# REXJJ/depth-map-fusion-utils

Measured on AMD Instinct MI355X. Metric: ray-voxel updates/sec (3D-DDA log-odds fusion, 512^3 grid, 640x480 depth), higher is better.
Workload: dtype int32

## Files before the change

### depth-map-fusion-utils_amd/csrc/dmf_brick.hpp

```cpp
#pragma once
#include <cmath>
#include <cstdint>

#ifndef __HIPCC__
#define __host__
#define __device__
#endif

namespace dmf {
namespace brick {

constexpr int kLog = 5;
constexpr int kB = 1 << kLog;
constexpr int kCells = kB * kB * kB;
constexpr int kMaxBricks = 32768;
constexpr int64_t kQ = 256;
constexpr int32_t kNever = 1 << 30;
constexpr int64_t kNever64 = (int64_t)1 << 62;

struct QRay {
  int32_t cs[3], ce[3];
  int32_t st[3];
  int32_t n[3];
  int32_t adq[3];
  int32_t h0[3];
  int32_t nsteps;
  bool end_inside;
};

__host__ __device__ inline void pack_ray(const int64_t qs[3], const int64_t qe[3], bool end_inside, uint64_t& A,
                                         uint64_t& B) {
  A = (uint64_t)qs[0] | ((uint64_t)qs[1] << 19) | ((uint64_t)qs[2] << 38) | ((uint64_t)(end_inside ? 1 : 0) << 63);
  B = (uint64_t)qe[0] | ((uint64_t)qe[1] << 19) | ((uint64_t)qe[2] << 38) | ((uint64_t)1 << 63);
}

__host__ __device__ inline void qray_from(const int32_t qs[3], const int32_t qe[3], bool end_inside, QRay& r) {
  r.end_inside = end_inside;
  r.nsteps = 0;
#pragma unroll
  for (int a = 0; a < 3; ++a) {
    r.cs[a] = qs[a] >> 8;
    r.ce[a] = qe[a] >> 8;
    const int32_t dq = qe[a] - qs[a];
    r.adq[a] = dq < 0 ? -dq : dq;
    r.st[a] = r.ce[a] > r.cs[a] ? 1 : (r.ce[a] < r.cs[a] ? -1 : 0);
    r.n[a] = r.ce[a] > r.cs[a] ? r.ce[a] - r.cs[a] : r.cs[a] - r.ce[a];
    r.h0[a] = r.st[a] > 0 ? 2 * ((r.cs[a] + 1) * (int32_t)kQ - qs[a]) : 2 * (qs[a] - r.cs[a] * (int32_t)kQ) + 1;
    r.nsteps += r.n[a];
  }
}

__host__ __device__ inline void decode_ray(uint64_t A, uint64_t B, QRay& r) {
  constexpr uint64_t m = (1u << 19) - 1;
  const int32_t qs[3] = {(int32_t)(A & m), (int32_t)((A >> 19) & m), (int32_t)((A >> 38) & m)};
  const int32_t qe[3] = {(int32_t)(B & m), (int32_t)((B >> 19) & m), (int32_t)((B >> 38) & m)};
  qray_from(qs, qe, (A >> 63) != 0, r);
}

__host__ __device__ inline int32_t e0_pair(const QRay& r, int a, int b) {
  if (r.st[a] && r.st[b]) return (int32_t)((int64_t)r.h0[a] * r.adq[b] - (int64_t)r.h0[b] * r.adq[a]);
  return r.st[a] ? -kNever : (r.st[b] ? kNever : 0);
}

__host__ __device__ inline bool ev_before(const QRay& r, int a, int64_t Ha, int b, int64_t Hb) {
  const int64_t L = Ha * (int64_t)r.adq[b], R = Hb * (int64_t)r.adq[a];
  return L < R || (L == R && a < b);
}

__host__ __device__ inline int32_t quot_small32(int64_t X, int32_t Y) {
  const float xf = (float)(int32_t)(X >> 20) * 1048576.0f + (float)(int32_t)(X & 0xfffff);
  const float yf = (float)Y;
#if defined(__HIP_DEVICE_COMPILE__)
  int32_t q = (int32_t)(xf * __builtin_amdgcn_rcpf(yf));
#else
  int32_t q = (int32_t)(xf / yf);
#endif
  const int32_t rm = (int32_t)((uint32_t)X - (uint32_t)q * (uint32_t)Y);
  q += rm < 0 ? -1 : (rm >= Y ? 1 : 0);
  return q;
}

__host__ __device__ inline int32_t count_at(const QRay& r, int b, int a, int32_t Ha) {
  if (r.st[b] == 0) return 0;
  const int64_t X = (int64_t)Ha * (int64_t)r.adq[b] - (int64_t)r.h0[b] * (int64_t)r.adq[a];
  const int32_t Y = (int32_t)(2 * kQ) * r.adq[a];
  int32_t c;
  if (b < a) c = X < 0 ? 0 : quot_small32(X, Y) + 1;
  else c = X <= 0 ? 0 : quot_small32(X - 1, Y) + 1;
  return c < r.n[b] ? c : r.n[b];
}

__host__ __device__ inline void counts_at(const QRay& r, int a, int32_t k, int32_t c[3]) {
  if (a < 0) { c[0] = c[1] = c[2] = 0; return; }
  const int32_t Ha = r.h0[a] + (int32_t)(2 * kQ) * k;
#pragma unroll
  for (int b = 0; b < 3; ++b) c[b] = (b == a) ? k + 1 : count_at(r, b, a, Ha);
}

__host__ __device__ inline int32_t opaque(int32_t x) {
#if defined(__HIP_DEVICE_COMPILE__)
  asm("" : "+v"(x));
#endif
  return x;
}

#if defined(__HIP_DEVICE_COMPILE__)
extern "C" __device__ int32_t dmf_llvm_mul_i24(int32_t, int32_t) __asm("llvm.amdgcn.mul.i24");
#endif
__host__ __device__ inline int32_t mul24(int32_t a, int32_t b) {
#if defined(__HIP_DEVICE_COMPILE__)
  return dmf_llvm_mul_i24(a, b);
#else
  return (int32_t)((uint32_t)a * (uint32_t)b);
#endif
}

__host__ __device__ inline int32_t sel3(bool a0, bool a1, int32_t v0, int32_t v1, int32_t v2) {
  return a0 ? opaque(v0) : (a1 ? opaque(v1) : opaque(v2));
}

__host__ __device__ inline void counts_at_sel(const QRay& r, int a, int32_t k, int32_t c[3]) {
  const bool a0 = a == 0, a1 = a == 1, a2 = a == 2;
  const int32_t ha = sel3(a0, a1, r.h0[0], r.h0[1], r.h0[2]);
  const int32_t da = sel3(a0, a1, r.adq[0], r.adq[1], r.adq[2]);
  const int64_t Ha = (int64_t)ha + 2 * kQ * (int64_t)k;
  const int32_t Y = (int32_t)(2 * kQ) * da;
  auto cnt = [&](int32_t adb, int32_t hb, int32_t nb, bool after) -> int32_t {
    const int64_t X = Ha * (int64_t)adb - (int64_t)hb * (int64_t)da - (after ? 1 : 0);
    const int32_t q = quot_small32(X < 0 ? 0 : X, Y) + 1;
    return X < 0 ? 0 : (q < 0 ? 0 : (q > nb ? nb : q));
  };
  const int32_t c1 = cnt(a0 ? opaque(r.adq[1]) : opaque(r.adq[0]), a0 ? opaque(r.h0[1]) : opaque(r.h0[0]),
// ... 10 lines not shown
  double hx[3][3];
};
__host__ __device__ inline void qray_f64(const QRay& r, QRayF64& f) {
#pragma unroll
  for (int a = 0; a < 3; ++a) {
    f.adq[a] = (double)r.adq[a];
    f.h[a] = (double)r.h0[a];
#if defined(__HIP_DEVICE_COMPILE__)
    f.inv[a] = r.adq[a] ? __builtin_amdgcn_rcp(2.0 * (double)kQ * (double)r.adq[a]) : 0.0;
#else
    f.inv[a] = r.adq[a] ? 1.0 / (2.0 * (double)kQ * (double)r.adq[a]) : 0.0;
#endif
  }
#pragma unroll
  for (int a = 0; a < 3; ++a)
#pragma unroll
    for (int b = 0; b < 3; ++b) f.hx[a][b] = -(f.h[b] * f.adq[a]) - (b > a ? 1.0 : 0.0);
}
template <int A>
__host__ __device__ inline void counts_at_f64(const QRay& r, const QRayF64& f, int32_t k, int32_t c[3]) {
  const double Ha = fma(2.0 * (double)kQ, (double)k, f.h[A]);
  const double Y = 2.0 * (double)kQ * f.adq[A];
#pragma unroll
  for (int b = 0; b < 3; ++b) {
    if (b == A) {
      c[b] = k + 1;
      continue;
    }
    const double X = fma(Ha, f.adq[b], f.hx[A][b]);
    const double q = floor(X * f.inv[A]);
    const double rm = fma(-q, Y, X);
    const int32_t cq = (int32_t)q + (rm < 0.0 ? 0 : 1) + (rm >= Y ? 1 : 0);
    c[b] = (r.st[b] == 0 || X < 0.0) ? 0 : (cq < r.n[b] ? cq : r.n[b]);
  }
}

struct Pair {
  int32_t cin[3];
  int32_t cells;
  bool ends;
};

__host__ __device__ inline void pair_in_brick(const QRay& r, const int32_t bb[3], const int32_t ng[3], Pair& p) {
  int ai = -1, ao = -1;
  int32_t ki = 0, ko = 0;
  int64_t Hi = 0, Ho = 0;
#pragma unroll
  for (int a = 0; a < 3; ++a) {
    const int32_t lo = bb[a] << kLog;
    const int32_t hi = (lo + kB - 1 < ng[a] - 1) ? lo + kB - 1 : ng[a] - 1;
    int32_t k = -1;
    if (r.st[a] > 0 && r.cs[a] < lo) k = lo - r.cs[a] - 1;
    if (r.st[a] < 0 && r.cs[a] > hi) k = r.cs[a] - hi - 1;
    if (k >= 0) {
      const int64_t H = (int64_t)r.h0[a] + 2 * kQ * (int64_t)k;
      if (ai < 0 || ev_before(r, ai, Hi, a, H)) { ai = a; ki = k; Hi = H; }
    }
    k = -1;
    if (r.st[a] > 0 && r.ce[a] > hi) k = hi - r.cs[a];
    if (r.st[a] < 0 && r.ce[a] < lo) k = r.cs[a] - lo;
    if (k >= 0) {
      const int64_t H = (int64_t)r.h0[a] + 2 * kQ * (int64_t)k;
      if (ao < 0 || ev_before(r, a, H, ao, Ho)) { ao = a; ko = k; Ho = H; }
    }
  }
  counts_at(r, ai, ki, p.cin);
  const int32_t idx_in = p.cin[0] + p.cin[1] + p.cin[2];
  if (ao >= 0) {
    int32_t co[3];
    counts_at(r, ao, ko, co);
    p.cells = co[0] + co[1] + co[2] - idx_in;
    p.ends = false;
  } else {
    p.cells = r.nsteps - idx_in + 1;
    p.ends = true;
  }
}

struct Coarse {
  int64_t E01, E02, E12, K0, K1, K2;
  int32_t total;
};

__host__ __device__ inline int32_t coarse_total(const QRay& r) {
  int32_t total = 0;
#pragma unroll
  for (int a = 0; a < 3; ++a) {
    const int32_t off = r.cs[a] & (kB - 1);
    const int32_t k0 = r.st[a] > 0 ? kB - 1 - off : off;
    if (r.st[a] != 0 && r.n[a] > k0) total += (r.n[a] - 1 - k0) / kB + 1;
  }
  return total;
}

__host__ __device__ inline void coarse_init(const QRay& r, Coarse& w) {
  int32_t H[3];
  w.total = coarse_total(r);
#pragma unroll
  for (int a = 0; a < 3; ++a) {
    const int32_t off = r.cs[a] & (kB - 1);
    const int32_t k0 = r.st[a] > 0 ? kB - 1 - off : off;
    H[a] = r.h0[a] + (int32_t)(2 * kQ) * k0;
  }
  auto pr = [&](int a, int b) -> int64_t {
    if (r.st[a] && r.st[b]) return (int64_t)H[a] * (int64_t)r.adq[b] - (int64_t)H[b] * (int64_t)r.adq[a];
    return r.st[a] ? -kNever64 : (r.st[b] ? kNever64 : 0);
  };
  w.E01 = pr(0, 1);
  w.E02 = pr(0, 2);
  w.E12 = pr(1, 2);
  w.K0 = (int64_t)kB * 2 * kQ * r.adq[0];
  w.K1 = (int64_t)kB * 2 * kQ * r.adq[1];
  w.K2 = (int64_t)kB * 2 * kQ * r.adq[2];
}

__host__ __device__ inline int coarse_next(Coarse& w) {
  const bool b10 = w.E01 > 0;
  const bool s2 = (b10 ? w.E12 : w.E02) > 0;
  const bool s1 = !s2 && b10, s0 = !s2 && !b10;
  w.E01 += s0 ? w.K1 : (s1 ? -w.K0 : 0);
  w.E02 += s0 ? w.K2 : (s2 ? -w.K0 : 0);
  w.E12 += s1 ? w.K2 : (s2 ? -w.K1 : 0);
  return s2 ? 2 : (s1 ? 1 : 0);
}

static_assert(kB * 2 * kQ == (1 << (kLog + 9)), "coarse K = 2^(kLog + 9) |dq|");
constexpr int kCoarseShift = kLog + 9;
constexpr int32_t kNever32 = 1 << 30;
struct Coarse32 {
  int32_t g01, g02, g12;
  int32_t d0, d1, d2;
  int32_t total;
};

__host__ __device__ inline void coarse_init32(const QRay& r, Coarse32& w) {
  int32_t H[3];
  w.total = coarse_total(r);
#pragma unroll
  for (int a = 0; a < 3; ++a) {
    const int32_t off = r.cs[a] & (kB - 1);
    const int32_t k0 = r.st[a] > 0 ? kB - 1 - off : off;
    H[a] = r.h0[a] + (int32_t)(2 * kQ) * k0;
  }
  auto pr = [&](int a, int b) -> int32_t {
    if (r.st[a] && r.st[b]) {
      auto mul = [](int32_t x, int32_t y) {
        return (int64_t)((uint64_t)((uint32_t)x & 0xffffffu) * ((uint32_t)y & 0xffffffu));
      };
      const int64_t E = mul(H[a], r.adq[b]) - mul(H[b], r.adq[a]);
      return (int32_t)((E - 1) >> kCoarseShift);
    }
    return r.st[a] ? -kNever32 : (r.st[b] ? kNever32 : -1);
  };
  w.g01 = pr(0, 1);
  w.g02 = pr(0, 2);
  w.g12 = pr(1, 2);
  w.d0 = r.adq[0];
  w.d1 = r.adq[1];
  w.d2 = r.adq[2];
}

__host__ __device__ inline int coarse_next32(Coarse32& w) {
  const bool b10 = w.g01 >= 0;
  const bool s2 = (b10 ? w.g12 : w.g02) >= 0;
  const bool s1 = !s2 && b10, s0 = !s2 && !b10;
  w.g01 += s0 ? w.d1 : (s1 ? -w.d0 : 0);
  w.g02 += s0 ? w.d2 : (s2 ? -w.d0 : 0);
  w.g12 += s1 ? w.d2 : (s2 ? -w.d1 : 0);
  return s2 ? 2 : (s1 ? 1 : 0);
}

__host__ __device__ inline bool coarse_gamma_ok(const QRay& r, const Coarse32& w) {
  auto ok = [&](int a, int b, int32_t g) {
    if (!r.st[a] || !r.st[b]) return true;
    const int32_t m = (r.adq[a] > r.adq[b] ? r.adq[a] : r.adq[b]) + 1;
    return g <= m && g >= -m;
  };
  return ok(0, 1, w.g01) && ok(0, 2, w.g02) && ok(1, 2, w.g12);
}

__host__ __device__ inline int32_t pinned(int32_t x) {
#if defined(__HIP_DEVICE_COMPILE__)
  asm volatile("" : "+v"(x));
#endif
  return x;
}
__host__ __device__ inline int coarse_next_k(const QRay& r, int32_t k0, int32_t k1, int32_t k2) {
  int best = -1;
  int64_t Hb = 0;
  int32_t db = 0;
  const int32_t ks[3] = {k0, k1, k2};
#pragma unroll
  for (int a = 0; a < 3; ++a) {
    const int32_t st = pinned(r.st[a]);
    if (st == 0) continue;
    const int32_t da = pinned(r.adq[a]);
    const int64_t H = (int64_t)pinned(r.h0[a]) + 2 * kQ * (int64_t)ks[a];
    if (best < 0 || H * (int64_t)db < Hb * (int64_t)da) {
      best = a;
      Hb = H;
      db = da;
    }
  }
  return best;
}
__host__ __device__ inline int32_t next_boundary_k(const QRay& r, int a, int b) {
  const int32_t st = r.st[a], nb = b + st;
  return st > 0 ? nb * kB - r.cs[a] - 1 : r.cs[a] - nb * kB - kB;
}
__host__ __device__ inline int coarse_next_at(const QRay& r, int b0, int b1, int b2) {
  return coarse_next_k(r, next_boundary_k(r, 0, b0), next_boundary_k(r, 1, b1), next_boundary_k(r, 2, b2));
}

constexpr int kPathSteps = 32;
__host__ __device__ inline uint64_t path_put(uint64_t path, int t, int a) {
  return t < kPathSteps ? path | (uint64_t)a << (2 * t) : path;
}
__host__ __device__ inline int path_axis(uint64_t path, int t) { return (int)(path >> (2 * t)) & 3; }
__host__ __device__ inline uint32_t path_word_put(uint32_t word, int t, int a) {
  return word | (uint32_t)a << ((2 * t) & 31);
}
__host__ __device__ inline int wave_uniform(int x) {
#if defined(__HIP_DEVICE_COMPILE__)
  return __builtin_amdgcn_readfirstlane(x);
// ... 231 lines not shown
```

### depth-map-fusion-utils_amd/csrc/dmf_dda.hpp

```cpp
#pragma once
#include "dmf_internal.hpp"

namespace dmf {

constexpr int64_t kQ = 256;

__device__ inline int64_t clampi(int64_t v, int64_t lo, int64_t hi) { return v < lo ? lo : (v > hi ? hi : v); }
__device__ inline int32_t clamp32(int32_t v, int32_t lo, int32_t hi) { return v < lo ? lo : (v > hi ? hi : v); }

__device__ inline int32_t floor_sat32(double x) {
  const double f = floor(x);
  return fabs(f) < 9223372036854775808.0 ? (int32_t)fmin(fmax(f, -1073741824.0), 1073741824.0) : -(1 << 30);
}

__device__ inline void atomic_add_dev(int32_t* p, int32_t v) {
  __hip_atomic_fetch_add(p, v, __ATOMIC_RELAXED, __HIP_MEMORY_SCOPE_AGENT);
}

struct Tiles {
  uint32_t ny, nz;
};
__host__ __device__ inline Tiles tiles_of(const int n[3]) {
  return Tiles{(uint32_t)(n[1] + 1) >> 1, (uint32_t)(n[2] + 3) >> 2};
}
__host__ __device__ inline uint32_t tile_base(const Tiles& t, int tx, int ty, int tz) {
  return (((uint32_t)tx * t.ny + (uint32_t)ty) * t.nz + (uint32_t)tz) << 4;
}
__host__ __device__ inline uint32_t tiled_index(const Tiles& t, int x, int y, int z) {
  return tile_base(t, x >> 1, y >> 1, z >> 2) | (uint32_t)(((x & 1) << 3) | ((y & 1) << 2) | (z & 3));
}
inline size_t tiled_cells(const int n[3]) {
  return (size_t)((n[0] + 1) >> 1) * (size_t)((n[1] + 1) >> 1) * (size_t)((n[2] + 3) >> 2) * 16;
}

struct Ray {
  int c[3];
  int st[3];
  int32_t E01, E02, E12;
  int32_t K[3];
  int left;
  bool end_inside;
};
constexpr int32_t kNever = 1 << 30;

__device__ inline void dda_select(int32_t& E01, int32_t& E02, int32_t& E12, int32_t K0, int32_t K1, int32_t K2,
                                  bool& s0, bool& s1, bool& s2) {
  const bool b10 = E01 > 0;
  s2 = (b10 ? E12 : E02) > 0;
  s1 = !s2 && b10;
  s0 = !s2 && !b10;
  E01 += s0 ? K1 : (s1 ? -K0 : 0);
  E02 += s0 ? K2 : (s2 ? -K0 : 0);
  E12 += s1 ? K2 : (s2 ? -K1 : 0);
}

struct Walk {
  int c0, c1, c2, st0, st1, st2;
  int32_t E01, E02, E12, K0, K1, K2;
  int left;
  __device__ explicit Walk(const Ray& R)
      : c0(R.c[0]), c1(R.c[1]), c2(R.c[2]), st0(R.st[0]), st1(R.st[1]), st2(R.st[2]), E01(R.E01), E02(R.E02),
        E12(R.E12), K0(R.K[0]), K1(R.K[1]), K2(R.K[2]), left(R.left) {}
  __device__ void step() {
    bool s0, s1, s2;
    dda_select(E01, E02, E12, K0, K1, K2, s0, s1, s2);
    c0 += s0 ? st0 : 0;
    c1 += s1 ? st1 : 0;
    c2 += s2 ? st2 : 0;
  }
};

__device__ inline double grid_coord(const Geom& g, int a, float x) {
  const double t = (double)x - g.mn[a];
  return g.pow2 ? t * g.inv[a] : t / g.dl[a];
}

__device__ inline void grid_origin(const Geom& g, const float O[3], double go[3]) {
#pragma unroll
  for (int a = 0; a < 3; ++a) go[a] = grid_coord(g, a, O[a]);
}

__device__ inline bool dda_quantize_go(const Geom& g, const double go[3], const float E[3], bool end_inside,
                                       int64_t qs[3], int64_t qe[3]) {
  double ge[3], D[3];
#pragma unroll
  for (int a = 0; a < 3; ++a) {
    ge[a] = grid_coord(g, a, E[a]);
    D[a] = ge[a] - go[a];
  }
  double t0 = 0.0, t1 = 1.0;
#pragma unroll
  for (int a = 0; a < 3; ++a) {
    if (D[a] == 0.0) {
      if (go[a] < 0.0 || go[a] >= (double)g.n[a]) return false;
    } else if (end_inside) {
      if (D[a] > 0.0 ? go[a] < 0.0 : go[a] > (double)g.n[a]) {
        const double lo = (D[a] > 0.0 ? 0.0 - go[a] : (double)g.n[a] - go[a]) / D[a];
        if (lo > t0) t0 = lo;
      }
    } else {
      double ta = (0.0 - go[a]) / D[a];
      double tb = ((double)g.n[a] - go[a]) / D[a];
      if (ta > tb) { const double tt = ta; ta = tb; tb = tt; }
      if (ta > t0) t0 = ta;
      if (tb < t1) t1 = tb;
    }
  }
  if (end_inside) { t1 = 1.0; if (t0 > 1.0) t0 = 1.0; }
  if (t0 > t1) return false;
#pragma unroll
  for (int a = 0; a < 3; ++a) {
    const double gs = go[a] + t0 * D[a];
    const double gx = end_inside ? ge[a] : go[a] + t1 * D[a];
    const int32_t n = (int32_t)g.n[a], Q = (int32_t)kQ;
    const int32_t cs = clamp32(floor_sat32(gs), 0, n - 1);
    const int32_t ce = end_inside ? floor_sat32(ge[a]) : clamp32(floor_sat32(gx), 0, n - 1);
    qs[a] = clamp32(floor_sat32(gs * (double)kQ), cs * Q, cs * Q + Q - 1);
    qe[a] = clamp32(floor_sat32(gx * (double)kQ), ce * Q, ce * Q + Q - 1);
  }
  return true;
}

__device__ inline bool dda_quantize(const Geom& g, const float O[3], const float E[3], bool end_inside, int64_t qs[3],
                                    int64_t qe[3]) {
  double go[3];
  grid_origin(g, O, go);
  return dda_quantize_go(g, go, E, end_inside, qs, qe);
}

__device__ inline bool dda_setup(const Geom& g, const float O[3], const float E[3], bool end_inside, Ray& R) {
  int64_t qs[3], qe[3];
  if (!dda_quantize(g, O, E, end_inside, qs, qe)) return false;
  int64_t cs[3], ce[3];
#pragma unroll
  for (int a = 0; a < 3; ++a) {
    cs[a] = qs[a] / kQ;
    ce[a] = qe[a] / kQ;
  }
  int64_t adq[3], h[3];
#pragma unroll
  for (int a = 0; a < 3; ++a) {
    const int64_t dq = qe[a] - qs[a];
    adq[a] = dq < 0 ? -dq : dq;
    R.st[a] = ce[a] > cs[a] ? 1 : (ce[a] < cs[a] ? -1 : 0);
    h[a] = R.st[a] > 0 ? 2 * ((cs[a] + 1) * kQ - qs[a]) : 2 * (qs[a] - cs[a] * kQ) + 1;
    R.K[a] = (int32_t)(2 * kQ * adq[a]);
  }
  auto pair = [&](int a, int b) -> int32_t {
    if (R.st[a] && R.st[b]) return (int32_t)(h[a] * adq[b] - h[b] * adq[a]);
    return R.st[a] ? -kNever : (R.st[b] ? kNever : 0);
  };
  R.E01 = pair(0, 1);
  R.E02 = pair(0, 2);
  R.E12 = pair(1, 2);
  const int nsteps = (int)((ce[0] > cs[0] ? ce[0] - cs[0] : cs[0] - ce[0]) + (ce[1] > cs[1] ? ce[1] - cs[1] : cs[1] - ce[1]) +
                           (ce[2] > cs[2] ? ce[2] - cs[2] : cs[2] - ce[2]));
  R.c[0] = (int)cs[0];
  R.c[1] = (int)cs[1];
  R.c[2] = (int)cs[2];
  R.left = nsteps + 1;
  R.end_inside = end_inside;
  return true;
}

__device__ inline bool endpoint_inside(const Geom& g, const float E[3]) {
  const bool in = (E[0] >= g.vlo[0]) & (E[0] <= g.vhi[0]) & (E[1] >= g.vlo[1]) & (E[1] <= g.vhi[1]) &
                  (E[2] >= g.vlo[2]) & (E[2] <= g.vhi[2]);
  if (!in) return false;
  return valid_coords(g, bin_axis(g, 0, E[0]), bin_axis(g, 1, E[1]), bin_axis(g, 2, E[2]));
}

__device__ inline int pixel_ray(const Geom& g, const CamP& cam, const uint16_t* __restrict__ depth,
                                const PoseX* __restrict__ poses, int p, int r, int c, int dmin, int dmax, Ray& R,
                                bool& valid) {
  R.left = 0;
  valid = false;
  if (r >= cam.H || c >= cam.W) return 0;
  const int d = depth[((int64_t)p * cam.H + r) * cam.W + c];
  if (!(d >= dmin && d < dmax)) return 0;
  valid = true;
  const PoseX& T = poses[p];
  float pc[3], E[3];
  project(cam, r, c, d, pc);
  xform(T.f, pc[0], pc[1], pc[2], E);
  const bool inside = endpoint_inside(g, E);
  const float O[3] = {T.f[3], T.f[7], T.f[11]};
  if (!dda_setup(g, O, E, inside, R)) { R.left = 0; return 0; }
  return R.left;
}

__device__ inline bool pixel_quant_go(const Geom& g, const CamP& cam, int d, const float Tf[12], const double go[3],
                                      int r, int c, int dmin, int dmax, int64_t qs[3], int64_t qe[3], bool& inside,
                                      bool& valid) {
  valid = false;
  inside = false;
  if (d < 0 || !(d >= dmin && d < dmax)) return false;
  valid = true;
  float pc[3], E[3];
  project(cam, r, c, d, pc);
  xform(Tf, pc[0], pc[1], pc[2], E);
  inside = endpoint_inside(g, E);
  return dda_quantize_go(g, go, E, inside, qs, qe);
}

__device__ inline int pixel_depth(const CamP& cam, const uint16_t* __restrict__ depth, int p, int r, int c) {
  return (r >= cam.H || c >= cam.W) ? -1 : (int)depth[((int64_t)p * cam.H + r) * cam.W + c];
}

__device__ inline int32_t rc_div(int64_t x, int32_t k) {
  int32_t q = (int32_t)((float)x * __builtin_amdgcn_rcpf((float)k));
  int64_t r = x - (int64_t)q * k;
  if (r < 0) { --q; r += k; }
  if (r < 0) { --q; r += k; }
  if (r >= k) { ++q; r -= k; }
  if (r >= k) { ++q; }
  return q;
}

__device__ inline int rc_jump(int m, Walk& W) {
  const int r0 = W.st0 > 0 ? m - (W.c0 & m) : (W.st0 < 0 ? (W.c0 & m) : 0);
  const int r1 = W.st1 > 0 ? m - (W.c1 & m) : (W.st1 < 0 ? (W.c1 & m) : 0);
  const int r2 = W.st2 > 0 ? m - (W.c2 & m) : (W.st2 < 0 ? (W.c2 & m) : 0);
  const int64_t F01 = (int64_t)W.E01 + (int64_t)r0 * W.K1 - (int64_t)r1 * W.K0;
  const int64_t F02 = (int64_t)W.E02 + (int64_t)r0 * W.K2 - (int64_t)r2 * W.K0;
  const int64_t F12 = (int64_t)W.E12 + (int64_t)r1 * W.K2 - (int64_t)r2 * W.K1;
  const bool b10 = F01 > 0;
  const bool s2 = (b10 ? F12 : F02) > 0, s1 = !s2 && b10;
  auto before = [](int64_t d, int rs, int32_t kb, int32_t ka, bool b_after) -> int {
    const int64_t x = d + (int64_t)rs * kb;
    if (x < 0 || ka == 0) return 0;
    const int32_t q = rc_div(x, ka);
    return b_after ? (int)(q + ((int64_t)q * ka < x ? 1 : 0)) : (int)q + 1;
  };
  int n0, n1, n2;
  if (s2) {
    n2 = r2 + 1;
    n0 = before(-(int64_t)W.E02, r2, W.K0, W.K2, false);
    n1 = before(-(int64_t)W.E12, r2, W.K1, W.K2, false);
  } else if (s1) {
    n1 = r1 + 1;
    n0 = before(-(int64_t)W.E01, r1, W.K0, W.K1, false);
    n2 = before((int64_t)W.E12, r1, W.K2, W.K1, true);
  } else {
    n0 = r0 + 1;
    n1 = before((int64_t)W.E01, r0, W.K1, W.K0, true);
    n2 = before((int64_t)W.E02, r0, W.K2, W.K0, true);
  }
  W.c0 += W.st0 * n0;
  W.c1 += W.st1 * n1;
  W.c2 += W.st2 * n2;
  W.E01 = (int32_t)((uint32_t)W.E01 + (uint32_t)n0 * (uint32_t)W.K1 - (uint32_t)n1 * (uint32_t)W.K0);
  W.E02 = (int32_t)((uint32_t)W.E02 + (uint32_t)n0 * (uint32_t)W.K2 - (uint32_t)n2 * (uint32_t)W.K0);
  W.E12 = (int32_t)((uint32_t)W.E12 + (uint32_t)n1 * (uint32_t)W.K2 - (uint32_t)n2 * (uint32_t)W.K1);
  return n0 + n1 + n2;
}

}
```

### depth-map-fusion-utils_amd/csrc/dmf_fuse.hip

```cpp
#include <algorithm>
#include <atomic>
#include <cmath>
#include <cstdlib>
#include <string>
#include <type_traits>

#include "dmf_brick.hpp"
#include "dmf_dda.hpp"
#include "dmf_host.hpp"

namespace dmf {

struct DepthSrc {
  CamP cam;
  const uint16_t* depth;
  const PoseX* poses;
  int dmin, dmax, packets_x;
  struct Frame { float Tf[12]; };
  struct Sample { int d, r, c; };
  __device__ void begin(const Geom& g, int p, Frame& f, double go[3]) const {
#pragma unroll
    for (int i = 0; i < 12; ++i) f.Tf[i] = poses[p].f[i];
    const float O[3] = {f.Tf[3], f.Tf[7], f.Tf[11]};
    grid_origin(g, O, go);
  }
  __device__ Sample load(int p, int q, int l) const {
    Sample s;
    s.r = (q / packets_x) * 8 + (l >> 3);
    s.c = (q % packets_x) * 8 + (l & 7);
    s.d = pixel_depth(cam, depth, p, s.r, s.c);
    return s;
  }
  __device__ bool quant(const Geom& g, const Frame& f, const double go[3], const Sample& s, int64_t qs[3],
                        int64_t qe[3], bool& inside, bool& valid) const {
    return pixel_quant_go(g, cam, s.d, f.Tf, go, s.r, s.c, dmin, dmax, qs, qe, inside, valid);
  }
  __device__ int ray(const Geom& g, int p, int q, int l, Ray& R, bool& valid) const {
    return pixel_ray(g, cam, depth, poses, p, (q / packets_x) * 8 + (l >> 3), (q % packets_x) * 8 + (l & 7), dmin,
                     dmax, R, valid);
  }
};

struct PointSrc {
  const float* xyz;
  const float* origins;
  int64_t N;
  struct Frame { bool live; };
  struct Sample { float E[3]; bool ok; };
  __device__ static bool finite3(const float v[3]) {
    return __builtin_isfinite(v[0]) & __builtin_isfinite(v[1]) & __builtin_isfinite(v[2]);
  }
  __device__ void origin(int p, float O[3]) const {
    const float* const o = origins + 3 * (int64_t)p;
    O[0] = o[0];
    O[1] = o[1];
    O[2] = o[2];
  }
  __device__ void begin(const Geom& g, int p, Frame& f, double go[3]) const {
    float O[3];
    origin(p, O);
    f.live = finite3(O);
    grid_origin(g, O, go);
  }
  __device__ Sample load(int p, int q, int l) const {
    Sample s;
    const int64_t i = (int64_t)q * 64 + l;
    s.ok = i < N;
    const float* const e = xyz + ((int64_t)p * N + (s.ok ? i : 0)) * 3;
    s.E[0] = e[0];
    s.E[1] = e[1];
    s.E[2] = e[2];
    return s;
  }
  __device__ bool quant(const Geom& g, const Frame& f, const double go[3], const Sample& s, int64_t qs[3],
                        int64_t qe[3], bool& inside, bool& valid) const {
    inside = false;
    valid = f.live & s.ok & finite3(s.E);
    if (!valid) return false;
    inside = endpoint_inside(g, s.E);
    return dda_quantize_go(g, go, s.E, inside, qs, qe);
  }
  __device__ int ray(const Geom& g, int p, int q, int l, Ray& R, bool& valid) const {
    float O[3];
    origin(p, O);
    const Sample s = load(p, q, l);
    R.left = 0;
    valid = finite3(O) && s.ok && finite3(s.E);
    if (!valid) return 0;
    if (!dda_setup(g, O, s.E, endpoint_inside(g, s.E), R)) { R.left = 0; return 0; }
    return R.left;
  }
};

__device__ inline void wave_stats(unsigned long long* stats, unsigned long long upd, unsigned long long ray,
                                  unsigned long long hit) {
  for (int o = 32; o > 0; o >>= 1) {
    upd += __shfl_down(upd, o, 64);
    ray += __shfl_down(ray, o, 64);
    hit += __shfl_down(hit, o, 64);
  }
  if ((threadIdx.x & 63) == 0) {
    if (upd) atomicAdd(&stats[0], upd);
    if (ray) atomicAdd(&stats[1], ray);
    if (hit) atomicAdd(&stats[2], hit);
  }
}


typedef unsigned short us2 __attribute__((ext_vector_type(2)));
__device__ inline uint32_t pkmax(uint32_t a, uint32_t b) {
  us2 x = __builtin_bit_cast(us2, a), y = __builtin_bit_cast(us2, b);
  return __builtin_bit_cast(uint32_t, __builtin_elementwise_max(x, y));
}
__device__ inline uint32_t wave_pkmax(uint32_t v) {
  v = pkmax(v, (uint32_t)__builtin_amdgcn_update_dpp(0, (int)v, 0x111, 0xf, 0xf, false));
  v = pkmax(v, (uint32_t)__builtin_amdgcn_update_dpp(0, (int)v, 0x112, 0xf, 0xf, false));
  v = pkmax(v, (uint32_t)__builtin_amdgcn_update_dpp(0, (int)v, 0x114, 0xf, 0xf, false));
  v = pkmax(v, (uint32_t)__builtin_amdgcn_update_dpp(0, (int)v, 0x118, 0xf, 0xf, false));
  v = pkmax(v, (uint32_t)__builtin_amdgcn_update_dpp(0, (int)v, 0x142, 0xa, 0xf, false));
  v = pkmax(v, (uint32_t)__builtin_amdgcn_update_dpp(0, (int)v, 0x143, 0xc, 0xf, false));
  return (uint32_t)__builtin_amdgcn_readlane((int)v, 63);
}

__device__ inline int lane_prefix(uint64_t mask) {
  return (int)__builtin_amdgcn_mbcnt_hi((uint32_t)(mask >> 32), __builtin_amdgcn_mbcnt_lo((uint32_t)mask, 0u));
}

__device__ inline int small_div(int i, int b, float rb, int& rem) {
  int q = (int)((float)i * rb);
  int r = i - q * b;
  if (r < 0) { --q; r += b; }
  if (r >= b) { ++q; r -= b; }
  rem = r;
  return q;
}

__device__ inline int popc(uint32_t v) { return __builtin_popcount(v); }
__device__ inline int popc(uint64_t v) { return __builtin_popcountll(v); }

template <int kS, int kBox, class Src>
__global__ __launch_bounds__(64) void k_fuse_l(Geom g, Src src, int32_t* __restrict__ hits,
                                               int32_t* __restrict__ misses,
                                               unsigned long long* __restrict__ stats) {
  static_assert(kS <= 31, "2-bit codes of up to 31 advances with a 64-bit field mask");
  using CodeT = typename std::conditional<(kS <= 15), uint32_t, uint64_t>::type;
  constexpr CodeT kOne = 1, kOdd = (CodeT)0x5555555555555555ull, kEven = (CodeT)0xAAAAAAAAAAAAAAAAull;
  static_assert(kBox % 256 == 0 && kBox <= 65536, "box scanned 256 cells per iteration, 16-bit indices");
  static_assert(kBox >= 64 * kS, "the non-zero list lives in the box");
  stats = stat_slot(stats);
  __shared__ __attribute__((aligned(16))) int box[kBox];
  uint32_t* nzl = (uint32_t*)box;
  const int l = threadIdx.x;
  for (int i = l; i < kBox; i += 64) box[i] = 0;
  const Tiles tl = tiles_of(g.n);
  Ray R;
  bool valid;
  const unsigned long long upd = (unsigned long long)src.ray(g, (int)blockIdx.y, (int)blockIdx.x, l, R, valid);
  const unsigned long long nvalid = valid ? 1 : 0, nhit = (R.left > 0 && R.end_inside) ? 1 : 0;
  int32_t E01 = R.E01, E02 = R.E02, E12 = R.E12;
  const int32_t K0 = R.K[0], K1 = R.K[1], K2 = R.K[2];
  const int st0 = R.st[0], st1 = R.st[1], st2 = R.st[2];
  int c0 = R.c[0], c1 = R.c[1], c2 = R.c[2], left = R.left;
  const bool end_inside = R.end_inside;
// ... 149 lines not shown

template <class F>
__device__ inline uint64_t bk_coarse(const BkGeom& bg, const bk::QRay& R, F&& f) {
  const int b = bk_index(bg, R.cs[0] >> bk::kLog, R.cs[1] >> bk::kLog, R.cs[2] >> bk::kLog);
  const int32_t D0 = bk::mul24(R.st[0], bg.nb[1] * bg.nb[2]), D1 = bk::mul24(R.st[1], bg.nb[2]), D2 = R.st[2];
  return bk::coarse_walk32(R, b, D0, D1, D2, f);
}

template <bool H16 = false>
__device__ inline void hist_add_first(uint32_t* hist, int b) {
  const int b0 = __builtin_amdgcn_readfirstlane(b);
  const uint64_t same = __builtin_amdgcn_ballot_w64(b == b0);
  const int l = (int)(threadIdx.x & 63);
  uint32_t* w;
  uint32_t n;
  if (b == b0) {
    if (l != __builtin_ctzll(same)) return;
    w = H16 ? &hist[b0 >> 1] : &hist[b0];
    n = (uint32_t)__builtin_popcountll(same);
  } else {
    w = H16 ? &hist[b >> 1] : &hist[b];
    n = 1u;
  }
  const int bb = b == b0 ? b0 : b;
  atomicAdd(w, H16 ? n << ((bb & 1) << 4) : n);
}

constexpr uint32_t kHashEmpty = 0xffff0000u;
__device__ inline bool hash_add(uint32_t* tab, uint32_t mask, int shift, uint32_t b, uint32_t n) {
  uint32_t h = (b * 2654435761u) >> shift;
  for (uint32_t k = 0; k <= mask; ++k) {
    const uint32_t old = atomicCAS(&tab[h], kHashEmpty, b << 16 | n);
    if (old == kHashEmpty) return true;
    if ((old >> 16) == b) {
      atomicAdd(&tab[h], n);
      return true;
    }
    h = (h + 1) & mask;
  }
  return false;
}

__device__ inline void hash_add_first(uint32_t* tab, uint32_t mask, int shift, int b, uint32_t* ovf) {
  const int b0 = __builtin_amdgcn_readfirstlane(b);
  const uint64_t same = __builtin_amdgcn_ballot_w64(b == b0);
  const int l = (int)(threadIdx.x & 63);
  if (b == b0 && l != __builtin_ctzll(same)) return;
  const uint32_t n = b == b0 ? (uint32_t)__builtin_popcountll(same) : 1u;
  if (!hash_add(tab, mask, shift, (uint32_t)b, n)) *ovf = 1u;
}

template <class Src>
struct BkRaysArgs {
  Geom g;
  Src src;
  int packets_pose, wg_pose, span;
  BkGeom bg;
  ulonglong2* rays;
  uint64_t* paths;
  uint32_t* pose_cnt;
  uint32_t* wg_base;
  uint32_t* wg_list;
  int wgl_stride;
  unsigned long long* pose_pairs;
  unsigned long long* stats;
  uint32_t* ovl;
  int hash_log;
};

template <bool H16, bool HASH, class Src>
__device__ inline void bk_rays_wg(const BkRaysArgs<Src>& A_, unsigned wg, uint32_t* hist, uint32_t* sh) {
  const Geom& g = A_.g;
  const BkGeom& bg = A_.bg;
  unsigned long long* const stats = stat_slot(A_.stats);
  const uint32_t hmask = (1u << A_.hash_log) - 1u;
  const int hshift = 32 - A_.hash_log;
  if (threadIdx.x == 0) {
    sh[0] = 0;
    sh[1] = 0;
  }
  const int nwords = HASH ? (int)hmask + 1 : (H16 ? (bg.nbricks + 1) >> 1 : bg.nbricks);
  for (int i = threadIdx.x; i < nwords; i += blockDim.x) hist[i] = HASH ? kHashEmpty : 0u;
  __syncthreads();
  const int w = threadIdx.x >> 6, l = threadIdx.x & 63, nw = blockDim.x >> 6;
  const int pw = (int)(wg / (unsigned)A_.wg_pose);
  const int q0 = (int)(wg - (unsigned)pw * (unsigned)A_.wg_pose) * A_.span;
  const int64_t pk0 = (int64_t)pw * A_.packets_pose + q0,
                pk1 = (int64_t)pw * A_.packets_pose + min(A_.packets_pose, q0 + A_.span);
  unsigned long long upd = 0, nvalid = 0, nhit = 0;
  double go[3];
  typename Src::Frame fr;
  A_.src.begin(g, pw, fr, go);
  for (int64_t pk = pk0 + w; pk < pk1; pk += nw) {
    const int p = pw;
    const int q = (int)(pk - (int64_t)p * A_.packets_pose);
    const typename Src::Sample sm = A_.src.load(p, q, l);
    int64_t qs[3], qe[3];
    bool inside, valid;
    ulonglong2 rec;
    rec.x = 0;
    rec.y = 0;
    uint64_t path = 0;
    if (A_.src.quant(g, fr, go, sm, qs, qe, inside, valid)) {
      uint64_t A, B;
      bk::pack_ray(qs, qe, inside, A, B);
      rec.x = A;
      rec.y = B;
      bk::QRay R;
      const int32_t qs32[3] = {(int32_t)qs[0], (int32_t)qs[1], (int32_t)qs[2]},
                    qe32[3] = {(int32_t)qe[0], (int32_t)qe[1], (int32_t)qe[2]};
      bk::qray_from(qs32, qe32, inside, R);
      upd += (unsigned long long)(R.nsteps + 1);
      nhit += inside ? 1 : 0;
      path = bk_coarse(bg, R, [&](int b) {
        if constexpr (HASH) hash_add_first(hist, hmask, hshift, b, &sh[1]);
        else hist_add_first<H16>(hist, b);
      });
    }
    nvalid += valid ? 1 : 0;
    A_.rays[pk * 64 + l] = rec;
    A_.paths[pk * 64 + l] = path;
  }
  __syncthreads();
  if (HASH && sh[1]) {
    if (threadIdx.x == 0) A_.ovl[1 + atomicAdd(&A_.ovl[0], 1u)] = wg;
    return;
  }
  uint32_t* const pc = A_.pose_cnt + (size_t)pw * bg.nbricks;
  uint32_t* const row = A_.wg_list + (size_t)wg * (size_t)A_.wgl_stride;
  unsigned long long mine = 0;
  for (int i = threadIdx.x; i < nwords; i += blockDim.x) {
    uint32_t b, n;
    if constexpr (HASH) {
      const uint32_t e = hist[i];
      b = e >> 16;
      n = e == kHashEmpty ? 0u : (e & 0xffffu);
    } else {
      b = (uint32_t)i;
      n = hist[i];
    }
    if (!HASH && H16) {
      for (int hh = 0; hh < 2; ++hh) {
        const uint32_t bb = 2u * (uint32_t)i + (uint32_t)hh, nn = (n >> (16 * hh)) & 0xffffu;
        if (nn) {
          A_.wg_base[(size_t)wg * bg.nbricks + bb] = atomicAdd(&pc[bb], nn);
          const uint32_t k = atomicAdd(&sh[0], 1u);
          row[1 + k] = bb | nn << 16;
          mine += nn;
        }
      }
    } else if (n) {
      A_.wg_base[(size_t)wg * bg.nbricks + b] = atomicAdd(&pc[b], n);
      const uint32_t k = atomicAdd(&sh[0], 1u);
      row[1 + k] = b | n << 16;
      mine += n;
    }
  }
  __syncthreads();
  if (threadIdx.x == 0) row[0] = sh[0];
  for (int o = 32; o > 0; o >>= 1) mine += __shfl_down(mine, o, 64);
  if (l == 0 && mine) atomicAdd(&A_.pose_pairs[pw], mine);
  if (stats) wave_stats(stats, upd, nvalid, nhit);
}

template <bool H16, class Src>
__global__ __launch_bounds__(kBkPassThreadsBig) void k_bk_rays(BkRaysArgs<Src> a) {
  extern __shared__ uint32_t hist[];
  __shared__ uint32_t sh[2];
  bk_rays_wg<H16, false>(a, blockIdx.x, hist, sh);
}

template <class Src>
__global__ __launch_bounds__(kBkPassThreads) void k_bk_rays_hash(BkRaysArgs<Src> a) {
  extern __shared__ uint32_t tab[];
  __shared__ uint32_t sh[2];
  bk_rays_wg<true, true>(a, blockIdx.x, tab, sh);
}

template <class Src>
__global__ __launch_bounds__(kBkPassThreadsBig) void k_bk_rays_recover(BkRaysArgs<Src> a) {
  extern __shared__ uint32_t hist[];
  __shared__ uint32_t sh[2];
  const uint32_t n = a.ovl[0];
  for (uint32_t i = blockIdx.x; i < n; i += gridDim.x) {
    bk_rays_wg<true, false>(a, a.ovl[1 + i], hist, sh);
    __syncthreads();
  }
}

__global__ __launch_bounds__(1024) void k_bk_batches(int P, const unsigned long long* __restrict__ pose_pairs,
                                                     unsigned long long cap, int max_poses,
                                                     uint32_t* __restrict__ bt) {
  constexpr int kChunk = 1024;
  __shared__ unsigned long long spp[kChunk];
  __shared__ unsigned long long s_tot;
  if (P <= max_poses) {
    if (threadIdx.x == 0) s_tot = 0;
    __syncthreads();
    unsigned long long part = 0;
    for (int i = (int)threadIdx.x; i < P; i += blockDim.x) part += pose_pairs[i];
    for (int o = 32; o > 0; o >>= 1) part += __shfl_down(part, o, 64);
    if ((threadIdx.x & 63) == 0 && part) atomicAdd(&s_tot, part);
    __syncthreads();
    if (s_tot <= cap) {
// ... 1739 lines not shown
```

Baseline: 1488 billion.

## Streamline ray quantization with 32-bit math and shared endpoint grid coords

Moves quantization into a new header and rewrites it to work in int32. The endpoint grid coordinate is computed once and reused for both the inside test and the clip. The floor/clamp chains become a hardware truncate-and-clamp to the grid extent, and qray setup uses v_sad_u32 with simpler sign and h0 formulas. Ray records are packed in 32-bit words and written as uint4, depth is loaded by block offsets, and the counters shrink to 32-bit. This cuts 64-bit and double-precision instruction count in the binning pass, at the risk of edge-case differences, since truncation is used instead of floor for negatives and the inside test is rewritten.

```diff
diff --git a/depth-map-fusion-utils_amd/csrc/dmf_brick.hpp b/depth-map-fusion-utils_amd/csrc/dmf_brick.hpp
--- a/depth-map-fusion-utils_amd/csrc/dmf_brick.hpp
+++ b/depth-map-fusion-utils_amd/csrc/dmf_brick.hpp
@@ -34,20 +34,40 @@
   B = (uint64_t)qe[0] | ((uint64_t)qe[1] << 19) | ((uint64_t)qe[2] << 38) | ((uint64_t)1 << 63);
 }
 
+__host__ __device__ inline void pack_ray32(const int32_t qs[3], const int32_t qe[3], bool end_inside, uint32_t a[2],
+                                           uint32_t b[2]) {
+  const uint32_t s0 = (uint32_t)qs[0], s1 = (uint32_t)qs[1], s2 = (uint32_t)qs[2];
+  const uint32_t e0 = (uint32_t)qe[0], e1 = (uint32_t)qe[1], e2 = (uint32_t)qe[2];
+  a[0] = s0 | s1 << 19;
+  a[1] = s1 >> 13 | s2 << 6 | (end_inside ? 1u << 31 : 0u);
+  b[0] = e0 | e1 << 19;
+  b[1] = e1 >> 13 | e2 << 6 | 1u << 31;
+}
+
+__host__ __device__ inline int32_t absdiff(int32_t x, int32_t y) {
+#if defined(__HIP_DEVICE_COMPILE__)
+  int32_t r;
+  asm("v_sad_u32 %0, %1, %2, 0" : "=v"(r) : "v"(x), "v"(y));
+  return r;
+#else
+  return x > y ? x - y : y - x;
+#endif
+}
+
 __host__ __device__ inline void qray_from(const int32_t qs[3], const int32_t qe[3], bool end_inside, QRay& r) {
   r.end_inside = end_inside;
-  r.nsteps = 0;
 #pragma unroll
   for (int a = 0; a < 3; ++a) {
     r.cs[a] = qs[a] >> 8;
     r.ce[a] = qe[a] >> 8;
-    const int32_t dq = qe[a] - qs[a];
-    r.adq[a] = dq < 0 ? -dq : dq;
-    r.st[a] = r.ce[a] > r.cs[a] ? 1 : (r.ce[a] < r.cs[a] ? -1 : 0);
-    r.n[a] = r.ce[a] > r.cs[a] ? r.ce[a] - r.cs[a] : r.cs[a] - r.ce[a];
-    r.h0[a] = r.st[a] > 0 ? 2 * ((r.cs[a] + 1) * (int32_t)kQ - qs[a]) : 2 * (qs[a] - r.cs[a] * (int32_t)kQ) + 1;
-    r.nsteps += r.n[a];
-  }
+    r.adq[a] = absdiff(qe[a], qs[a]);
+    const int32_t d = r.ce[a] - r.cs[a];
+    r.st[a] = d < -1 ? -1 : (d > 1 ? 1 : d);
+    r.n[a] = absdiff(r.ce[a], r.cs[a]);
+    const int32_t f2 = 2 * (qs[a] & ((int32_t)kQ - 1));
+    r.h0[a] = d > 0 ? 2 * (int32_t)kQ - f2 : f2 + 1;
+  }
+  r.nsteps = r.n[0] + r.n[1] + r.n[2];
 }
 
 __host__ __device__ inline void decode_ray(uint64_t A, uint64_t B, QRay& r) {
@@ -224,14 +244,17 @@
   int32_t total;
 };
 
+__host__ __device__ inline int32_t first_boundary(const QRay& r, int a) {
+  const int32_t off = r.cs[a] & (kB - 1);
+  return r.ce[a] - r.cs[a] > 0 ? kB - 1 - off : off;
+}
+
+__host__ __device__ inline int32_t boundaries_from(int32_t n, int32_t k0) { return (n + (kB - 1 - k0)) >> kLog; }
+
 __host__ __device__ inline int32_t coarse_total(const QRay& r) {
   int32_t total = 0;
 #pragma unroll
-  for (int a = 0; a < 3; ++a) {
-    const int32_t off = r.cs[a] & (kB - 1);
-    const int32_t k0 = r.st[a] > 0 ? kB - 1 - off : off;
-    if (r.st[a] != 0 && r.n[a] > k0) total += (r.n[a] - 1 - k0) / kB + 1;
-  }
+  for (int a = 0; a < 3; ++a) total += boundaries_from(r.n[a], first_boundary(r, a));
   return total;
 }
 
@@ -277,11 +300,11 @@
 
 __host__ __device__ inline void coarse_init32(const QRay& r, Coarse32& w) {
   int32_t H[3];
-  w.total = coarse_total(r);
+  w.total = 0;
 #pragma unroll
   for (int a = 0; a < 3; ++a) {
-    const int32_t off = r.cs[a] & (kB - 1);
-    const int32_t k0 = r.st[a] > 0 ? kB - 1 - off : off;
+    const int32_t k0 = first_boundary(r, a);
+    w.total += boundaries_from(r.n[a], k0);
     H[a] = r.h0[a] + (int32_t)(2 * kQ) * k0;
   }
   auto pr = [&](int a, int b) -> int32_t {
diff --git a/depth-map-fusion-utils_amd/csrc/dmf_dda.hpp b/depth-map-fusion-utils_amd/csrc/dmf_dda.hpp
--- a/depth-map-fusion-utils_amd/csrc/dmf_dda.hpp
+++ b/depth-map-fusion-utils_amd/csrc/dmf_dda.hpp
@@ -1,17 +1,9 @@
 #pragma once
 #include "dmf_internal.hpp"
+#include "dmf_quant.hpp"
 
 namespace dmf {
 
-constexpr int64_t kQ = 256;
-
-__device__ inline int64_t clampi(int64_t v, int64_t lo, int64_t hi) { return v < lo ? lo : (v > hi ? hi : v); }
-__device__ inline int32_t clamp32(int32_t v, int32_t lo, int32_t hi) { return v < lo ? lo : (v > hi ? hi : v); }
-
-__device__ inline int32_t floor_sat32(double x) {
-  const double f = floor(x);
-  return fabs(f) < 9223372036854775808.0 ? (int32_t)fmin(fmax(f, -1073741824.0), 1073741824.0) : -(1 << 30);
-}
 
 __device__ inline void atomic_add_dev(int32_t* p, int32_t v) {
   __hip_atomic_fetch_add(p, v, __ATOMIC_RELAXED, __HIP_MEMORY_SCOPE_AGENT);
@@ -70,67 +62,13 @@
   }
 };
 
-__device__ inline double grid_coord(const Geom& g, int a, float x) {
-  const double t = (double)x - g.mn[a];
-  return g.pow2 ? t * g.inv[a] : t / g.dl[a];
-}
-
-__device__ inline void grid_origin(const Geom& g, const float O[3], double go[3]) {
-#pragma unroll
-  for (int a = 0; a < 3; ++a) go[a] = grid_coord(g, a, O[a]);
-}
-
-__device__ inline bool dda_quantize_go(const Geom& g, const double go[3], const float E[3], bool end_inside,
-                                       int64_t qs[3], int64_t qe[3]) {
-  double ge[3], D[3];
-#pragma unroll
-  for (int a = 0; a < 3; ++a) {
-    ge[a] = grid_coord(g, a, E[a]);
-    D[a] = ge[a] - go[a];
-  }
-  double t0 = 0.0, t1 = 1.0;
-#pragma unroll
-  for (int a = 0; a < 3; ++a) {
-    if (D[a] == 0.0) {
-      if (go[a] < 0.0 || go[a] >= (double)g.n[a]) return false;
-    } else if (end_inside) {
-      if (D[a] > 0.0 ? go[a] < 0.0 : go[a] > (double)g.n[a]) {
-        const double lo = (D[a] > 0.0 ? 0.0 - go[a] : (double)g.n[a] - go[a]) / D[a];
-        if (lo > t0) t0 = lo;
-      }
-    } else {
-      double ta = (0.0 - go[a]) / D[a];
-      double tb = ((double)g.n[a] - go[a]) / D[a];
-      if (ta > tb) { const double tt = ta; ta = tb; tb = tt; }
-      if (ta > t0) t0 = ta;
-      if (tb < t1) t1 = tb;
-    }
-  }
-  if (end_inside) { t1 = 1.0; if (t0 > 1.0) t0 = 1.0; }
-  if (t0 > t1) return false;
-#pragma unroll
-  for (int a = 0; a < 3; ++a) {
-    const double gs = go[a] + t0 * D[a];
-    const double gx = end_inside ? ge[a] : go[a] + t1 * D[a];
-    const int32_t n = (int32_t)g.n[a], Q = (int32_t)kQ;
-    const int32_t cs = clamp32(floor_sat32(gs), 0, n - 1);
-    const int32_t ce = end_inside ? floor_sat32(ge[a]) : clamp32(floor_sat32(gx), 0, n - 1);
-    qs[a] = clamp32(floor_sat32(gs * (double)kQ), cs * Q, cs * Q + Q - 1);
-    qe[a] = clamp32(floor_sat32(gx * (double)kQ), ce * Q, ce * Q + Q - 1);
-  }
-  return true;
-}
-
-__device__ inline bool dda_quantize(const Geom& g, const float O[3], const float E[3], bool end_inside, int64_t qs[3],
-                                    int64_t qe[3]) {
-  double go[3];
+__device__ inline bool dda_setup(const Geom& g, const float O[3], const float E[3], bool end_inside, Ray& R) {
+  double go[3], ge[3];
   grid_origin(g, O, go);
-  return dda_quantize_go(g, go, E, end_inside, qs, qe);
-}
-
-__device__ inline bool dda_setup(const Geom& g, const float O[3], const float E[3], bool end_inside, Ray& R) {
-  int64_t qs[3], qe[3];
-  if (!dda_quantize(g, O, E, end_inside, qs, qe)) return false;
+  grid_origin(g, E, ge);
+  int32_t qs32[3], qe32[3];
+  if (!dda_quantize_ge(g, go, ge, end_inside, qs32, qe32)) return false;
+  const int64_t qs[3] = {qs32[0], qs32[1], qs32[2]}, qe[3] = {qe32[0], qe32[1], qe32[2]};
   int64_t cs[3], ce[3];
 #pragma unroll
   for (int a = 0; a < 3; ++a) {
@@ -163,13 +101,6 @@
   return true;
 }
 
-__device__ inline bool endpoint_inside(const Geom& g, const float E[3]) {
-  const bool in = (E[0] >= g.vlo[0]) & (E[0] <= g.vhi[0]) & (E[1] >= g.vlo[1]) & (E[1] <= g.vhi[1]) &
-                  (E[2] >= g.vlo[2]) & (E[2] <= g.vhi[2]);
-  if (!in) return false;
-  return valid_coords(g, bin_axis(g, 0, E[0]), bin_axis(g, 1, E[1]), bin_axis(g, 2, E[2]));
-}
-
 __device__ inline int pixel_ray(const Geom& g, const CamP& cam, const uint16_t* __restrict__ depth,
                                 const PoseX* __restrict__ poses, int p, int r, int c, int dmin, int dmax, Ray& R,
                                 bool& valid) {
@@ -190,7 +121,7 @@
 }
 
 __device__ inline bool pixel_quant_go(const Geom& g, const CamP& cam, int d, const float Tf[12], const double go[3],
-                                      int r, int c, int dmin, int dmax, int64_t qs[3], int64_t qe[3], bool& inside,
+                                      int r, int c, int dmin, int dmax, int32_t qs[3], int32_t qe[3], bool& inside,
                                       bool& valid) {
   valid = false;
   inside = false;
@@ -199,8 +130,7 @@
   float pc[3], E[3];
   project(cam, r, c, d, pc);
   xform(Tf, pc[0], pc[1], pc[2], E);
-  inside = endpoint_inside(g, E);
-  return dda_quantize_go(g, go, E, inside, qs, qe);
+  return dda_quantize_go(g, go, E, &inside, qs, qe);
 }
 
 __device__ inline int pixel_depth(const CamP& cam, const uint16_t* __restrict__ depth, int p, int r, int c) {
diff --git a/depth-map-fusion-utils_amd/csrc/dmf_fuse.hip b/depth-map-fusion-utils_amd/csrc/dmf_fuse.hip
--- a/depth-map-fusion-utils_amd/csrc/dmf_fuse.hip
+++ b/depth-map-fusion-utils_amd/csrc/dmf_fuse.hip
@@ -26,13 +26,16 @@
   }
   __device__ Sample load(int p, int q, int l) const {
     Sample s;
-    s.r = (q / packets_x) * 8 + (l >> 3);
-    s.c = (q % packets_x) * 8 + (l & 7);
-    s.d = pixel_depth(cam, depth, p, s.r, s.c);
+    const int qy = q / packets_x, r0 = qy * 8, c0 = (q - qy * packets_x) * 8;
+    s.r = r0 + (l >> 3);
+    s.c = c0 + (l & 7);
+    const uint16_t* const block = depth + (((int64_t)p * cam.H + r0) * cam.W + c0);
+    const uint32_t off = (uint32_t)(l >> 3) * (uint32_t)cam.W + (uint32_t)(l & 7);
+    s.d = (s.r >= cam.H || s.c >= cam.W) ? -1 : (int)block[off];
     return s;
   }
-  __device__ bool quant(const Geom& g, const Frame& f, const double go[3], const Sample& s, int64_t qs[3],
-                        int64_t qe[3], bool& inside, bool& valid) const {
+  __device__ bool quant(const Geom& g, const Frame& f, const double go[3], const Sample& s, int32_t qs[3],
+                        int32_t qe[3], bool& inside, bool& valid) const {
     return pixel_quant_go(g, cam, s.d, f.Tf, go, s.r, s.c, dmin, dmax, qs, qe, inside, valid);
   }
   __device__ int ray(const Geom& g, int p, int q, int l, Ray& R, bool& valid) const {
@@ -72,13 +75,12 @@
     s.E[2] = e[2];
     return s;
   }
-  __device__ bool quant(const Geom& g, const Frame& f, const double go[3], const Sample& s, int64_t qs[3],
-                        int64_t qe[3], bool& inside, bool& valid) const {
+  __device__ bool quant(const Geom& g, const Frame& f, const double go[3], const Sample& s, int32_t qs[3],
+                        int32_t qe[3], bool& inside, bool& valid) const {
     inside = false;
     valid = f.live & s.ok & finite3(s.E);
     if (!valid) return false;
-    inside = endpoint_inside(g, s.E);
-    return dda_quantize_go(g, go, s.E, inside, qs, qe);
+    return dda_quantize_go(g, go, s.E, &inside, qs, qe);
   }
   __device__ int ray(const Geom& g, int p, int q, int l, Ray& R, bool& valid) const {
     float O[3];
@@ -394,12 +396,12 @@
   const int nwords = HASH ? (int)hmask + 1 : (H16 ? (bg.nbricks + 1) >> 1 : bg.nbricks);
   for (int i = threadIdx.x; i < nwords; i += blockDim.x) hist[i] = HASH ? kHashEmpty : 0u;
   __syncthreads();
-  const int w = threadIdx.x >> 6, l = threadIdx.x & 63, nw = blockDim.x >> 6;
+  const int w = bk::wave_uniform((int)(threadIdx.x >> 6)), l = threadIdx.x & 63, nw = blockDim.x >> 6;
   const int pw = (int)(wg / (unsigned)A_.wg_pose);
   const int q0 = (int)(wg - (unsigned)pw * (unsigned)A_.wg_pose) * A_.span;
   const int64_t pk0 = (int64_t)pw * A_.packets_pose + q0,
                 pk1 = (int64_t)pw * A_.packets_pose + min(A_.packets_pose, q0 + A_.span);
-  unsigned long long upd = 0, nvalid = 0, nhit = 0;
+  uint32_t upd = 0, nvalid = 0, nhit = 0;
   double go[3];
   typename Src::Frame fr;
   A_.src.begin(g, pw, fr, go);
@@ -407,22 +409,17 @@
     const int p = pw;
     const int q = (int)(pk - (int64_t)p * A_.packets_pose);
     const typename Src::Sample sm = A_.src.load(p, q, l);
-    int64_t qs[3], qe[3];
+    int32_t qs[3], qe[3];
     bool inside, valid;
-    ulonglong2 rec;
-    rec.x = 0;
-    rec.y = 0;
+    uint4 rec = make_uint4(0u, 0u, 0u, 0u);
     uint64_t path = 0;
     if (A_.src.quant(g, fr, go, sm, qs, qe, inside, valid)) {
-      uint64_t A, B;
-      bk::pack_ray(qs, qe, inside, A, B);
-      rec.x = A;
-      rec.y = B;
+      uint32_t ra[2], rb[2];
+      bk::pack_ray32(qs, qe, inside, ra, rb);
+      rec = make_uint4(ra[0], ra[1], rb[0], rb[1]);
       bk::QRay R;
-      const int32_t qs32[3] = {(int32_t)qs[0], (int32_t)qs[1], (int32_t)qs[2]},
-                    qe32[3] = {(int32_t)qe[0], (int32_t)qe[1], (int32_t)qe[2]};
-      bk::qray_from(qs32, qe32, inside, R);
-      upd += (unsigned long long)(R.nsteps + 1);
+      bk::qray_from(qs, qe, inside, R);
+      upd += (uint32_t)(R.nsteps + 1);
       nhit += inside ? 1 : 0;
       path = bk_coarse(bg, R, [&](int b) {
         if constexpr (HASH) hash_add_first(hist, hmask, hshift, b, &sh[1]);
@@ -430,8 +427,8 @@
       });
     }
     nvalid += valid ? 1 : 0;
-    A_.rays[pk * 64 + l] = rec;
-    A_.paths[pk * 64 + l] = path;
+    reinterpret_cast<uint4*>(A_.rays + pk * 64)[l] = rec;
+    (A_.paths + pk * 64)[l] = path;
   }
   __syncthreads();
   if (HASH && sh[1]) {
diff --git a/depth-map-fusion-utils_amd/csrc/dmf_quant.hpp b/depth-map-fusion-utils_amd/csrc/dmf_quant.hpp
--- /dev/null
+++ b/depth-map-fusion-utils_amd/csrc/dmf_quant.hpp
@@ -0,0 +1,122 @@
+#pragma once
+#include <cmath>
+#include <cstdint>
+
+#include "dmf_geom.hpp"
+
+namespace dmf {
+
+constexpr int64_t kQ = 256;
+
+__host__ __device__ inline int32_t imin32(int32_t a, int32_t b) { return a < b ? a : b; }
+__host__ __device__ inline int32_t imax32(int32_t a, int32_t b) { return a > b ? a : b; }
+
+__host__ __device__ inline int32_t trunc_sat32(double x) {
+#if defined(__HIP_DEVICE_COMPILE__)
+  int32_t r;
+  asm("v_cvt_i32_f64 %0, %1" : "=v"(r) : "v"(x));
+  return r;
+#else
+  if (!(x == x)) return 0;
+  if (x <= -2147483648.0) return INT32_MIN;
+  if (x >= 2147483647.0) return INT32_MAX;
+  return (int32_t)x;
+#endif
+}
+
+__host__ __device__ inline void keep_branch() {
+#if defined(__HIP_DEVICE_COMPILE__)
+  asm volatile("");
+#endif
+}
+
+__host__ __device__ inline double grid_coord(const Geom& g, int a, float x) {
+  const double t = (double)x - g.mn[a];
+  return g.pow2 ? t * g.inv[a] : t / g.dl[a];
+}
+
+__host__ __device__ inline void grid_origin(const Geom& g, const float O[3], double go[3]) {
+#pragma unroll
+  for (int a = 0; a < 3; ++a) go[a] = grid_coord(g, a, O[a]);
+}
+
+__host__ __device__ inline bool endpoint_inside_ge(const Geom& g, const float E[3], const double ge[3]) {
+  const bool in = (E[0] >= g.vlo[0]) & (E[0] <= g.vhi[0]) & (E[1] >= g.vlo[1]) & (E[1] <= g.vhi[1]) &
+                  (E[2] >= g.vlo[2]) & (E[2] <= g.vhi[2]);
+  return in & (ge[0] >= 0.0) & (ge[0] < (double)g.n[0]) & (ge[1] >= 0.0) & (ge[1] < (double)g.n[1]) &
+         (ge[2] >= 0.0) & (ge[2] < (double)g.n[2]);
+}
+__host__ __device__ inline bool endpoint_inside(const Geom& g, const float E[3]) {
+  double ge[3];
+  grid_origin(g, E, ge);
+  return endpoint_inside_ge(g, E, ge);
+}
+
+__host__ __device__ inline int32_t quant_far(double y, int32_t top) {
+  return y < 9223372036854775808.0 ? top : (y < 2361183241434822606848.0 ? top - ((int32_t)kQ - 1) : 0);
+}
+__host__ __device__ inline int32_t quant_coord(double x, int32_t top) {
+  const double y = x * (double)kQ;
+  const int32_t i = trunc_sat32(y);
+  int32_t q = imin32(imax32(i, 0), top);
+  if (i == INT32_MAX) {
+    keep_branch();
+    q = quant_far(y, top);
+  }
+  return q;
+}
+
+__host__ __device__ inline bool dda_quantize_ge(const Geom& g, const double go[3], const double ge[3], bool end_inside,
+                                                int32_t qs[3], int32_t qe[3]) {
+  double D[3];
+#pragma unroll
+  for (int a = 0; a < 3; ++a) D[a] = ge[a] - go[a];
+  double t0 = 0.0, t1 = 1.0;
+#pragma unroll
+  for (int a = 0; a < 3; ++a) {
+    if (D[a] == 0.0) {
+      if (go[a] < 0.0 || go[a] >= (double)g.n[a]) return false;
+    } else if (end_inside) {
+      if (D[a] > 0.0 ? go[a] < 0.0 : go[a] > (double)g.n[a]) {
+        const double lo = (D[a] > 0.0 ? 0.0 - go[a] : (double)g.n[a] - go[a]) / D[a];
+        if (lo > t0) t0 = lo;
+      }
+    } else {
+      double ta = (0.0 - go[a]) / D[a];
+      double tb = ((double)g.n[a] - go[a]) / D[a];
+      if (ta > tb) { const double tt = ta; ta = tb; tb = tt; }
+      if (ta > t0) t0 = ta;
+      if (tb < t1) t1 = tb;
+    }
+  }
+  if (end_inside) { t1 = 1.0; if (t0 > 1.0) t0 = 1.0; }
+  if (t0 > t1) return false;
+  double gs[3], gx[3];
+#pragma unroll
+  for (int a = 0; a < 3; ++a) {
+    gs[a] = go[a] + t0 * D[a];
+    gx[a] = ge[a];
+  }
+  if (!end_inside) {
+    keep_branch();
+#pragma unroll
+    for (int a = 0; a < 3; ++a) gx[a] = go[a] + t1 * D[a];
+  }
+#pragma unroll
+  for (int a = 0; a < 3; ++a) {
+    const int32_t top = (int32_t)g.n[a] * (int32_t)kQ - 1;
+    qs[a] = quant_coord(gs[a], top);
+    qe[a] = quant_coord(gx[a], top);
+  }
+  return true;
+}
+
+__host__ __device__ inline bool dda_quantize_go(const Geom& g, const double go[3], const float E[3], bool* inside,
+                                                int32_t qs[3], int32_t qe[3]) {
+  double ge[3];
+  grid_origin(g, E, ge);
+  *inside = endpoint_inside_ge(g, E, ge);
+  return dda_quantize_ge(g, go, ge, *inside, qs, qe);
+}
+
+}
```

Measured after the change: 1515 billion (median of 6 runs). 1.02x the previous value.
